# refresh-bio/KMC

Measured on AMD Instinct MI355X. Metric: stage-2 Gk-mers/s, k=27, higher is better.
Workload: dtype u64

## Files before the change

### kmc_amd/csrc/bucket_sort.hip.h

```cpp
#ifndef KMC_AMD_BUCKET_SORT_HIP_H
#define KMC_AMD_BUCKET_SORT_HIP_H

#include "kernels.hip.h"

#ifndef BR_NARROW_LOOP
#define BR_NARROW_LOOP 2
#endif
#ifndef BR_WIDE_LOOP
#define BR_WIDE_LOOP 1
#endif
#ifndef BR_WIDE_STEP
#define BR_WIDE_STEP 8
#endif
#ifndef BR_SLACK_DIV
#define BR_SLACK_DIV 12
#endif
#ifndef BR_INDIRECT_MIN_SIZE
#define BR_INDIRECT_MIN_SIZE 2
#endif
#ifndef BR_MIN_WAVES
#define BR_MIN_WAVES 6
#endif
template <int SIZE> __device__ __forceinline__ u64 bs_p64(const u64 (&x)[SIZE], u32 key_bits)
{
// ... 759 lines not shown
						s_aux[j] = (u32)kmc_remove_suffix<1>(kx, pshift) & lut_mask;
				}
				__syncthreads();
				for (u32 w = tid; w < ndw; w += THREADS) {
					const u32 i0 = w << 2;
					u32 ri = rec_bytes > 1 ? __umulhi(i0, inv) : i0, q = i0 - ri * rec_bytes;
					u64 cur = s_key[ri];
					u32 word = 0;
#pragma unroll
					for (int t = 0; t < 4; ++t) {
						word |= ((u32)(cur >> (8 * q)) & 0xFFu) << (8 * t);
						if (++q == rec_bytes) {
							q = 0;
							++ri;
							cur = s_key[ri < (u32)CAP ? ri : (u32)CAP - 1];
						}
					}
					dst32[w] = word;
				}
				if (use_lut) {
					u64 *lut = gr.lut_base[bin] + (size_t)(slot % lut_shards) * lut_stride;
					for (u32 j = tid; j < tile_counted; j += THREADS) {
						const u32 pf = s_aux[j];
						if (j + 1 == tile_counted || s_aux[j + 1] != pf)
							atomicAdd(&lut[pf], (u64)(j + 1));
						if (j > 0 && s_aux[j - 1] != pf)
							atomicAdd(&lut[pf], (u64)0 - (u64)j);
					}
				}
			} else {
#pragma unroll
				for (int r = 0; r < ITEMS; ++r) {
					const u32 rk16 = (rank2[r >> 1] >> ((r & 1) * 16)) & 0xFFFFu;
					if (rk16 != 0xFFFFu) {
						const u32 rank = wave_off + rk16;
						u64 kx[SIZE];
#pragma unroll
						for (int w = 0; w < SIZE; ++w)
							kx[w] = key[r][w];
						kmc_mask_low<SIZE>(kx, 2 * P.k);
						store_rec<SIZE>(s_key + (size_t)rank * SIZE, kx);
						s_aux[rank] = cnt[r];
					}
				}
				__syncthreads();
				auto out_byte = [&](u32 i) -> u32 {
					const u32 ri = rec_bytes > 1 ? __umulhi(i, inv) : i, q = i - ri * rec_bytes;
					if (q < P.sbytes) {
						const u32 pbyte = P.sbytes - 1 - q;
						return (u32)(s_key[(size_t)ri * SIZE + (pbyte >> 3)] >> ((pbyte & 7) * 8)) & 0xFFu;
					}
					const u32 cq = q - P.sbytes;
					return (s_aux[ri] >> (8 * (P.kff ? (P.cbytes - 1 - cq) : cq))) & 0xFFu;
				};
#pragma clang loop unroll(disable) vectorize(disable)
				for (u32 wd = tid; wd < ndw; wd += THREADS) {
					const u32 i0 = wd * 4;
					u32 word = out_byte(i0);
					word |= (i0 + 1 < tile_bytes ? out_byte(i0 + 1) : 0u) << 8;
					word |= (i0 + 2 < tile_bytes ? out_byte(i0 + 2) : 0u) << 16;
					word |= (i0 + 3 < tile_bytes ? out_byte(i0 + 3) : 0u) << 24;
					dst32[wd] = word;
				}
				if (use_lut) {
					u64 *lut = gr.lut_base[bin] + (size_t)(slot % lut_shards) * lut_stride;
					auto prefix_of = [&](u32 j) -> u32 {
						u64 x[SIZE];
						load_rec<SIZE>(s_key + (size_t)j * SIZE, x);
						return (u32)kmc_remove_suffix<SIZE>(x, pshift) & lut_mask;
					};
					for (u32 j = tid; j < tile_counted; j += THREADS) {
						const u32 pf = prefix_of(j);
						if (j + 1 == tile_counted || prefix_of(j + 1) != pf)
							atomicAdd(&lut[pf], (u64)(j + 1));
						if (j > 0 && prefix_of(j - 1) != pf)
							atomicAdd(&lut[pf], (u64)0 - (u64)j);
					}
				}
			}
		}
	}
}

template <int SIZE, bool FUSED>
__global__ void __launch_bounds__(BrCfg<SIZE>::THREADS, BR_MIN_WAVES) k_bucket_rank(const GrpRank gr, DevParams P, u32 key_bits, u32 hbits, u32 lut_shards, u64 lut_stride,
                                                                                  u32 lut_mask, u32 *flag)
{
	KMC_DYN_LDS(unsigned char, s_raw);
	br_tile<SIZE, FUSED>(gr, P, key_bits, hbits, lut_shards, lut_stride, lut_mask, flag, blockIdx.x, blockIdx.y, s_raw);
}

template <int SIZE>
__global__ void __launch_bounds__(GT_THREADS) k_giant_tiles(const GrpRank gr, DevParams P, u32 stride, u32 key_bits, u32 hbits, u32 lut_shards, u64 lut_stride, u32 lut_mask,
                                                              u32 *err )
{
	constexpr int THREADS = GT_THREADS, ITEMS = SIZE == 1 ? 8 : (SIZE == 2 ? 4 : 2), NW = THREADS / 64, CHUNK = THREADS * ITEMS;
	constexpr u32 NONE = 0xFFFFFFFFu;
	static_assert(THREADS >= 256, "one digit per thread");
	__shared__ u32 s_whist[NW * 256];
	__shared__ u32 s_base[256];
	__shared__ u32 s_scan[NW + 1];
	__shared__ u32 s_pick;
	__shared__ u32 s_wlast[NW], s_wcnt[NW];
	const u32 tid = threadIdx.x, lane = tid & 63;
	const u32 wave = (u32)__builtin_amdgcn_readfirstlane((int)(tid >> 6));
	const u32 rec_bytes = P.sbytes + P.cbytes;
	const bool use_lut = P.lut_prefix_len != 0 && !P.kff && !P.without_output;
	const u32 pshift = 2 * (P.k - P.lut_prefix_len);
	const u32 bsh = 64 - hbits, rbits = key_bits - hbits;
	const u64 lane_lt = (1ull << lane) - 1;
	while (true) {
		__syncthreads();
		if (tid == 0)
			s_pick = atomicAdd(&gr.giant[1], 1u);
		__syncthreads();
		const u32 pick = s_pick;
		if (pick >= ld_agent(&gr.giant[0]))
			break;
		const u32 entry = gr.giant[2 + pick];
		const u32 gtile = entry & ((1u << GT_CUT_SHIFT) - 1u), cut = entry >> GT_CUT_SHIFT;
		const u32 bin = (u32)__builtin_amdgcn_readfirstlane((int)grp_find(gr.win_prefix, gr.g, gtile));
		const u32 tile = gtile - gr.win_prefix[bin];
		const u64 b0 = gr.bounds[bin][tile] + cut, b1 = gr.bounds[bin][tile + 1];
		const u32 L = (u32)(b1 - b0);
		u64 *T = gr.S[bin] + b0 * SIZE;
		if (gr.rec_base) {
			T = gr.giant_T[bin] + b0 * SIZE;
			const u64 *pairs = gr.S[bin] + b0;
			for (u32 i = tid; i < L; i += THREADS) {
				u64 x[SIZE];
				load_rec<SIZE>(gr.rec_base + (size_t)(u32)pairs[i] * SIZE, x);
				store_rec<SIZE>(T + (size_t)i * SIZE, x);
			}
			__syncthreads();
		}
		u64 *U = reinterpret_cast<u64 *>(gr.scratch[bin] + b0 * (u64)(SIZE * 8));
		(void)stride;
		u32 passes;
		{
			u64 x0[SIZE], xl[SIZE];
			load_rec<SIZE>(T, x0);
			load_rec<SIZE>(T + (size_t)(L - 1) * SIZE, xl);
			const u64 k0 = hbits ? bs_p64<SIZE>(x0, key_bits) >> bsh : 0ull, kl = hbits ? bs_p64<SIZE>(xl, key_bits) >> bsh : 0ull;
			const u64 diff = k0 ^ kl;
			const u32 dbits = diff ? 64u - (u32)__clzll((long long)diff) : 0u;
			const u32 nbits = rbits + dbits < key_bits ? rbits + dbits : key_bits;
			passes = (nbits + 7) / 8;
		}
		u64 *src = T, *dst = U;
		for (u32 p = 0; p < passes; ++p) {
			if (tid < 256)
				s_base[tid] = 0;
			__syncthreads();
			for (u32 i = tid; i < L; i += THREADS) {
				u64 x[SIZE];
				load_rec<SIZE>(src + (size_t)i * SIZE, x);
				(void)__hip_atomic_fetch_add(&s_base[kmc_get_byte<SIZE>(x, p)], 1u, __ATOMIC_RELAXED, __HIP_MEMORY_SCOPE_WORKGROUP);
			}
			__syncthreads();
			{
				const u32 v = tid < 256 ? s_base[tid] : 0u;
				u32 total;
				const u32 ex = block_excl_sum<NW, u32>(v, s_scan, total);
				if (tid < 256)
					s_base[tid] = ex;
			}
			__syncthreads();
			for (u32 c0 = 0; c0 < L; c0 += CHUNK) {
				for (u32 i = tid; i < (u32)NW * 256; i += THREADS)
					s_whist[i] = 0;
				__syncthreads();
				u64 key[ITEMS][SIZE];
// ... 188 lines not shown
```

### kmc_amd/csrc/host_plan_and_groups.hip.h

```cpp
u32 lut_shards_for(u64 lut_entries) { return lut_entries <= 256 ? 32u : (lut_entries <= 1024 ? 8u : 1u); }

struct BinPlan {
	const uint8_t *d_in = nullptr;
	u64 size = 0, n_rec = 0, n_packs = 0;
	const u64 *d_pack_start = nullptr;
	uint8_t *d_out = nullptr;
	u64 out_capacity = 0;
	u64 *d_out_bytes = nullptr, *d_lut = nullptr, *d_stats = nullptr;
	size_t off_bitmap = 0, off_exp_status = 0, off_cp_status = 0, off_lutsh = 0, off_tally = 0;
	u64 rec_off = 0;
};

struct SortPlan {
	u32 key_bytes = 0, top = 0;
	u32 key_bits = 0;
	bool rank = false;
	u32 pass_lo() const { return key_bytes - top; }
	bool local() const { return top < key_bytes; }
	u32 hbits() const { return top ? 8 * top - (8 * key_bytes - key_bits) : 0; }
};
std::atomic<u64> g_path[4] = {};
std::atomic<u64> g_indirect_groups{0};
std::atomic<u64> g_hybrid_groups{0}, g_redo_groups{0};
std::atomic<u32> g_extra_top{0};
// ... 57 lines not shown
	if (n <= (u64)BrCfg<SIZE>::THREADS * (8 / SIZE > 2 ? 8 / SIZE : 2))
		return sp;
	const u64 redo = g_redo_groups.load(std::memory_order_relaxed);
	if (g_extra_top.load(std::memory_order_relaxed) >= 2 && redo > 128 && redo * 8 > g_hybrid_groups.load(std::memory_order_relaxed))
		return sp;
	for (u32 h = 1; h + 2 <= key_bytes && h <= 6u; ++h) {
		const u32 eff = 8 * h > spare ? 8 * h - spare : 0;
		if (eff >= 28 && (eff >= 63 || (n >> eff) <= 2) && key_bits - eff <= rem_limit) {
			sp.top = h;
			break;
		}
	}
	if (sp.top + 2 > key_bytes)
		sp.top = key_bytes;
	static const int forced = [] {
		const char *e = getenv("KMC_HIP_RANK_TOP");
		return e ? atoi(e) : 0;
	}();
	if (forced >= 1 && (u32)forced + 1 <= key_bytes && 8 * (u32)forced > spare)
		sp.top = (u32)forced;
	if (sp.local() && sp.top >= 1 && key_bits - sp.hbits() <= rem_limit && sp.hbits() <= 48)
		sp.rank = true;
	else
		sp.top = key_bytes;
	return sp;
}

template <int SIZE>
ZeroPlan plan_group(const Slot &s, std::vector<BinPlan> &bins, u64 n_total, u32 n_pass , bool front, bool sort, bool compact, u64 lut_shard_entries,
                    u64 cp_tile = CpCfg<SIZE>::TILE ,
                    u32 cp_words = 1 , u64 giant_entries = 0, bool arena = false)
{
	ZeroPlan z;
	size_t off = up256(SM_BYTES);
	if (giant_entries) {
		z.giant = off;
		off += up256((size_t)(giant_entries + 2) * 4);
	}
	if (arena) {
		z.arena = off;
		off += up256((size_t)AR_DYN_WORDS * 4) + up256((size_t)AR_MAX_PASS * 256 * 8);
	}
	for (BinPlan &b : bins) {
		if (front) {
			b.off_bitmap = off;
			off += up256(((b.size + 31) / 32 + 2) * 4);
			b.off_exp_status = off;
			off += up256(((b.size + EXP_CHUNK - 1) / EXP_CHUNK) * 8 + 8);
		}
		if (compact) {
			b.off_cp_status = off;
			off += up256(((b.n_rec + cp_tile - 1) / cp_tile) * 8 * cp_words + 8);
			b.off_lutsh = off;
			off += up256(lut_shard_entries * 8);
			b.off_tally = off;
			off += up256(CP_SHARDS * 4 * 8);
		}
	}
	if (front || sort) {
		z.ghist = off;
		off += up256((size_t)n_pass * 256 * 8);
	}
	if (sort && n_total >= 2) {
		const u64 max_tiles = (std::min(n_total, s.portion) + RsCfg<SIZE>::TILE - 1) / RsCfg<SIZE>::TILE;
		const u64 n_launch = (u64)n_pass * ((n_total + s.portion - 1) / s.portion);
		z.sc_status = off;
		z.sc_stride = up256((size_t)max_tiles * 256 * 4);
		off += z.sc_stride * n_launch;
	}
	z.total = off;
	return z;
}

int apply_plan(Slot &s, const ZeroPlan &z)
{
	s.zero_grew = z.total > s.zero.cap;
	++s.groups_run;
	if (int rc = ensure(s.zero, z.total))
		return rc;
	HIPCHK(hipMemsetAsync(s.zero.p, 0, z.total, s.stream));
	return 0;
}

template <int SIZE>
int sort_device_t(Slot &s, const ZeroPlan &z, u64 *d_recs, u64 *d_tmp, u64 n, const SortPlan &sp, u64 **d_result, u32 &counter_idx, bool hist_done, u32 *d_flag,
                  bool local_by_caller = false )
{
	u64 *src = d_recs, *dst = d_tmp;
	if (n < 2 || sp.key_bytes == 0) {
		*d_result = src;
		if (s.timed)
			HIPCHK(hipEventRecord(s.ev[3], s.stream));
		return 0;
	}
	const u32 n_pass = sp.top, pass_lo = sp.pass_lo();
	u32 *err = err_ptr(s);
	if (n_pass) {
		if (int rc = ensure(s.dbase, (size_t)n_pass * 256 * 8))
			return rc;
		u64 *ghist = zero_ptr<u64>(s, z.ghist), *dbase = (u64 *)s.dbase.p;
		u32 *counters = small_ptr<u32>(s, SM_COUNTERS);
		u64 *work = small_ptr<u64>(s, SM_DBASE_WORK);

		if (!hist_done) {
			u64 blocks = (n + 255) / 256;
			if (blocks > 256 * 8)
				blocks = 256 * 8;
			k_hist<SIZE><<<dim3((u32)blocks), dim3(256), (size_t)n_pass * 1024, s.stream>>>(src, n, n_pass, ghist, pass_lo);
			k_hist_scan<<<dim3(n_pass), dim3(256), 0, s.stream>>>(ghist, dbase);
		}
		if (s.timed)
			HIPCHK(hipEventRecord(s.ev[3], s.stream));
		u32 launch = 0;
		for (u32 pass = 0; pass < n_pass; ++pass) {
			const u64 *base_in = dbase + (size_t)pass * 256;
			int flip = 0;
			for (u64 start = 0; start < n; start += s.portion) {
				const u32 cnt = (u32)std::min(s.portion, n - start);
				const u32 tiles = (cnt + RsCfg<SIZE>::TILE - 1) / RsCfg<SIZE>::TILE;
				if (counter_idx >= N_COUNTERS)
					return fail(KMC_HIP_EINVAL, "too many scatter launches for one bin");
				u32 *status = zero_ptr<u32>(s, z.sc_status + (size_t)launch * z.sc_stride);
				u64 *base_out = work + (size_t)flip * 256;
				hipEvent_t e0 = nullptr, e1 = nullptr;
				if (s.timed) {
					if (int rc = sc_event_pair(s, e0, e1, cnt))
						return rc;
					HIPCHK(hipEventRecord(e0, s.stream));
				}
				static const size_t scatter_pad = [] {
					const char *e = getenv("KMC_HIP_SCATTER_LDS_PAD");
					const size_t v = e ? (size_t)strtoull(e, nullptr, 10) : (size_t)0;
					return v > 32 * 1024 ? (size_t)32 * 1024 : v;
				}();
				k_onesweep<SIZE><<<dim3((tiles + RS_TPB - 1) / RS_TPB), dim3(RS_BLOCK), rs_lds_bytes<SIZE>() + scatter_pad, s.stream>>>(
				    src + start * SIZE, dst, cnt, pass_lo + pass, base_in, base_out, status, counters + counter_idx, tiles, err);
				if (s.timed)
					HIPCHK(hipEventRecord(e1, s.stream));
				++counter_idx;
				++launch;
				base_in = base_out;
				flip ^= 1;
			}
			std::swap(src, dst);
		}
	} else if (s.timed)
		HIPCHK(hipEventRecord(s.ev[3], s.stream));
	if (sp.local() && !local_by_caller) {
		if constexpr (SIZE == 1) {
			if (!sp.rank)
				return fail(KMC_HIP_EINTERNAL, "a local sort plan without the rank finisher");
			const u64 S = (u64)BrCfg<1>::STRIDE;
			const u64 n_win = (n + S - 1) / S;
			if (n_win > 0x7FFFFFF0ull)
				return fail(KMC_HIP_EINVAL, "bin too large");
			if (int rc = ensure(s.bounds, (size_t)(n_win + 2) * 8))
				return rc;
			u64 *bounds = (u64 *)s.bounds.p;
			hipEvent_t e0 = nullptr, e1 = nullptr;
			if (s.timed) {
				if (int rc = ls_event_pair(s, e0, e1, n))
					return rc;
				HIPCHK(hipEventRecord(e0, s.stream));
			}
			GrpBounds gbn = {};
			gbn.g = 1;
			gbn.item_prefix[1] = (u32)(n_win + 1);
			gbn.S[0] = src;
			gbn.n[0] = n;
			gbn.bounds[0] = bounds;
			k_bucket_bounds<1><<<dim3((u32)((n_win + 1 + 3) / 4)), dim3(256), 0, s.stream>>>(gbn, (u32)S, sp.key_bits, sp.hbits());
			GrpRank gr = {};
			gr.g = 1;
			gr.win_prefix[1] = (u32)n_win;
			gr.S[0] = src;
			gr.bounds[0] = bounds;
			k_bucket_rank<1, false><<<dim3((u32)n_win, 2), dim3(BrCfg<1>::THREADS), br_lds_bytes<1>(), s.stream>>>(gr, DevParams{}, sp.key_bits, sp.hbits(), 1u, 0ull, 0u, d_flag);
			if (s.timed)
				HIPCHK(hipEventRecord(e1, s.stream));
		} else
			return fail(KMC_HIP_EINTERNAL, "records of two words and more have no in-place local sort");
	}
	HIPCHK(hipGetLastError());
	*d_result = src;
	return 0;
}

template <int SIZE> int sort_only_t(Slot &s, u64 *d_recs, u64 *d_tmp, u64 n, u32 key_bytes, u64 **d_result, bool stable_lsd)
{
	std::vector<BinPlan> none;
	const SortPlan sp = plan_sort<SIZE>(n, key_bytes, 8 * key_bytes, stable_lsd);
	const ZeroPlan z = plan_group<SIZE>(s, none, n, sp.top, false, true, false, 0);
	if (int rc = apply_plan(s, z))
		return rc;
	u32 counter_idx = 0;
	return sort_device_t<SIZE>(s, z, d_recs, d_tmp, n, sp, d_result, counter_idx, false, small_ptr<u32>(s, SM_REDO));
}

int sort_device(Slot &s, u64 *d_recs, u64 *d_tmp, u64 n, u32 words, u32 n_pass, u64 **d_result, bool stable_lsd)
{
	return by_words<8>(words, [&](auto W) { return sort_only_t<decltype(W)::value>(s, d_recs, d_tmp, n, n_pass, d_result, stable_lsd); });
}

int check_params(const kmc_hip_bin_params *p, DevParams &P)
{
	if (!p)
		return fail(KMC_HIP_EINVAL, "params == NULL");
	if (p->kmer_len < 1 || p->kmer_len > 256)
		return fail(KMC_HIP_EINVAL, "kmer_len must be 1..256");
	if (p->output_type > 1)
		return fail(KMC_HIP_EINVAL, "output_type must be 0 (KMC) or 1 (KFF)");
	if (p->lut_prefix_len >= p->kmer_len && p->lut_prefix_len)
		return fail(KMC_HIP_EINVAL, "lut_prefix_len must be < kmer_len");
	if (p->lut_prefix_len > 15)
		return fail(KMC_HIP_EINVAL, "lut_prefix_len must be <= 15");
	if (p->lut_prefix_len && (p->kmer_len - p->lut_prefix_len) % 4)
		return fail(KMC_HIP_EINVAL, "(kmer_len - lut_prefix_len) must be a multiple of 4 (kmc.h:1454-1456)");
	P.k = p->kmer_len;
	P.both_strands = p->both_strands ? 1 : 0;
	P.cutoff_min = p->cutoff_min;
	P.cutoff_max = (u32)p->cutoff_max;
	P.counter_max = (u32)p->counter_max;
	P.lut_prefix_len = p->lut_prefix_len;
	P.sbytes = kmc_suffix_bytes(p->kmer_len, p->lut_prefix_len);
	P.cbytes = counter_bytes(p->cutoff_max, p->counter_max);
	P.kff = p->output_type == 1;
	P.without_output = p->without_output ? 1 : 0;
	return 0;
}

template <int SIZE>
int front_end_group(Slot &s, const std::vector<BinPlan> &bins, size_t off_ghist, const DevParams &P, u32 n_pass , u32 pass_lo, u32 &counter_idx,
                    bool &hist_done, u64 *d_recs, bool fuse, u64 *d_pairs = nullptr )
{
	if (bins.empty())
		return 0;
	if (bins.size() > (size_t)GRP_MAX)
		return fail(KMC_HIP_EINVAL, "group too large");
	u32 *err = err_ptr(s);
	u32 *counters = small_ptr<u32>(s, SM_COUNTERS);
	if (counter_idx + 2 > N_COUNTERS)
		return fail(KMC_HIP_EINVAL, "too many launches for one bin");
	GrpParse gp = {};
	GrpExpand ge = {};
	gp.g = ge.g = (u32)bins.size();
	u64 packs = 0, chunks = 0;
	const u32 tag_shift = (2 * P.k) & 63;
	for (size_t i = 0; i < bins.size(); ++i) {
		const BinPlan &b = bins[i];
		gp.pack_prefix[i] = (u32)packs;
		ge.chunk_prefix[i] = (u32)chunks;
		packs += b.n_packs;
		chunks += (b.size + EXP_CHUNK - 1) / EXP_CHUNK;
		if (packs > 0x7FFFFFF0ull || chunks > 0x7FFFFFF0ull)
			return fail(KMC_HIP_EINVAL, "bin too large");
		gp.data[i] = ge.data[i] = b.d_in;
		gp.pack_start[i] = b.d_pack_start;
		gp.bitmap[i] = zero_ptr<u32>(s, b.off_bitmap);
		ge.bitmap[i] = gp.bitmap[i];
		ge.size[i] = b.size;
// ... 9 lines not shown
	u64 *ghist = zero_ptr<u64>(s, off_ghist);
	k_parse_packs<<<dim3((u32)packs), dim3(PARSE_BLOCK), 0, s.stream>>>(gp, P.k, err);
	if (s.timed)
		HIPCHK(hipEventRecord(s.ev[1], s.stream));
	const u32 blocks = (u32)std::min<u64>(chunks, 256 * 4 * (512 / EXP_BLOCK));
	if (fuse) {
		if (int rc = ensure(s.dbase, (size_t)n_pass * 256 * 8))
			return rc;
		k_expand<SIZE, true><<<dim3(blocks), dim3(EXP_BLOCK), exp_lds_bytes<true>(n_pass, P.k), s.stream>>>(
		    ge, P.k, P.both_strands, n_pass, ghist, counters + counter_idx, err, (u64 *)s.dbase.p, counters + counter_idx + 1, pass_lo);
	} else
		k_expand<SIZE, false><<<dim3(blocks), dim3(EXP_BLOCK), exp_lds_bytes<false>(n_pass, P.k), s.stream>>>(
		    ge, P.k, P.both_strands, n_pass, ghist, counters + counter_idx, err, nullptr, counters + counter_idx + 1, pass_lo);
	counter_idx += 2;
	hist_done = fuse;
	if (s.timed)
		HIPCHK(hipEventRecord(s.ev[2], s.stream));
	HIPCHK(hipGetLastError());
	return 0;
}

template <int SIZE>
int compact_group(Slot &s, const std::vector<BinPlan> &bins, const u64 *sorted, u64 *scratch, const DevParams &P, u64 lut_entries, u32 &counter_idx)
{
	if (bins.empty())
		return 0;
	u32 *err = err_ptr(s);
	u32 *counters = small_ptr<u32>(s, SM_COUNTERS);
	if (counter_idx >= N_COUNTERS)
		return fail(KMC_HIP_EINVAL, "too many launches for one bin");
	const bool use_lut = lut_entries && !P.without_output && !P.kff;
	const u32 n_sh = !use_lut ? 1u : lut_shards_for(lut_entries);
	const u32 rec_bytes = P.sbytes + P.cbytes;
	const u64 tile_pitch = (u64)CpCfg<SIZE>::TILE * SIZE * 8;
	static const bool allow_two_phase = [] {
		const char *e = getenv("KMC_HIP_TWO_PHASE");
		return !e || atoi(e) != 0;
	}();
	const bool two_phase = allow_two_phase && scratch && !P.without_output &&
	                       ((u64)CpCfg<SIZE>::TILE / std::max<u32>(P.cutoff_min, 1) + 1) * rec_bytes <= tile_pitch;
	GrpCompact gc = {};
	GrpFold gf = {};
	GrpGather gg = {};
	gc.g = gg.g = (u32)bins.size();
	u64 tiles = 0;
	for (size_t i = 0; i < bins.size(); ++i) {
		const BinPlan &b = bins[i];
		gc.tile_prefix[i] = gg.tile_prefix[i] = (u32)tiles;
		const u64 bin_tiles = (b.n_rec + CpCfg<SIZE>::TILE - 1) / CpCfg<SIZE>::TILE;
		tiles += bin_tiles;
		if (tiles > 0x7FFFFFFFull)
			return fail(KMC_HIP_EINVAL, "bin too large");
		u64 *lut_base = b.d_lut;
		if (use_lut && n_sh > 1)
			lut_base = zero_ptr<u64>(s, b.off_lutsh);
		else if (lut_entries && !P.kff && b.d_lut)
			HIPCHK(hipMemsetAsync(b.d_lut, 0, lut_entries * 8, s.stream));
		gc.S[i] = sorted + b.rec_off * SIZE;
		gc.n[i] = gf.n[i] = b.n_rec;
		gc.out[i] = b.d_out;
		gc.out_capacity[i] = b.out_capacity;
		gc.lut_base[i] = lut_base;
		gc.tally[i] = zero_ptr<u64>(s, b.off_tally);
		gc.out_bytes[i] = b.d_out_bytes;
		gc.status[i] = zero_ptr<u64>(s, b.off_cp_status);
		gf.tally[i] = gc.tally[i];
		gf.stats[i] = b.d_stats;
		gf.lut_base[i] = lut_base;
		gf.lut_out[i] = b.d_lut;
		gc.scratch[i] = two_phase ? (uint8_t *)(scratch + b.rec_off * SIZE) : nullptr;
		gf.status[i] = gc.status[i];
		gf.n_tiles[i] = (u32)bin_tiles;
		gf.out_bytes[i] = b.d_out_bytes;
		gf.out_capacity[i] = b.out_capacity;
		gg.scratch[i] = gc.scratch[i];
		gg.prefix[i] = gc.status[i];
		gg.out[i] = b.d_out;
		gg.out_capacity[i] = b.out_capacity;
	}
	gc.tile_prefix[bins.size()] = gg.tile_prefix[bins.size()] = (u32)tiles;
	k_compact<SIZE><<<dim3((u32)tiles), dim3(CP_BLOCK), 0, s.stream>>>(gc, P, n_sh, lut_entries, counters + counter_idx, err,
	                                                                   P.lut_prefix_len ? (u32)((1ull << (2 * P.lut_prefix_len)) - 1) : 0u, two_phase ? 1u : 0u);
	counter_idx += 1;
	k_compact_fold<<<dim3((u32)bins.size()), dim3(256), 0, s.stream>>>(gf, use_lut ? n_sh : 1u, lut_entries, two_phase ? 1u : 0u, rec_bytes, err);
	if (two_phase)
		k_compact_gather<<<dim3((u32)((tiles + 3) / 4)), dim3(256), 0, s.stream>>>(gg, rec_bytes, tile_pitch);
	HIPCHK(hipGetLastError());
	return 0;
}

template <int SIZE> bool count_applicable(const DevParams &P)
{
	static const bool allow_two_phase = [] {
		const char *e = getenv("KMC_HIP_TWO_PHASE");
		return !e || atoi(e) != 0;
	}();
	const u32 rec_bytes = P.sbytes + P.cbytes;
	return allow_two_phase && (P.without_output || rec_bytes <= (u32)(SIZE * 8));
}
template <int SIZE>
int rank_group(Slot &s, const std::vector<BinPlan> &bins, u64 *sorted, u64 *scratch, const DevParams &P, u64 lut_entries, const SortPlan &sp, u64 n_total, u32 *d_flag,
               u32 *d_giant, const u64 *d_recs_indirect = nullptr ,
               u32 *d_arena = nullptr )
{
	if (bins.empty())
		return 0;
	u32 *err = err_ptr(s);
	const bool use_lut = lut_entries && !P.without_output && !P.kff;
	const u32 n_sh = !use_lut ? 1u : lut_shards_for(lut_entries);
	const u32 rec_bytes = P.sbytes + P.cbytes;
	constexpr u64 S = BrCfg<SIZE>::STRIDE;
	GrpBounds gbn = {};
	GrpRank gr = {};
	GrpFold gf = {};
	GrpGather gg = {};
	gbn.g = gr.g = gg.g = (u32)bins.size();
	u64 wins = 0, items = 0;
	for (const BinPlan &b : bins) {
		items += (b.n_rec + S - 1) / S + 1;
		wins += (b.n_rec + S - 1) / S;
	}
	if (items > 0x3FFFFFF0ull)
		return fail(KMC_HIP_EINVAL, "bin too large");
	if (int rc = ensure(s.bounds, (size_t)(items + 2 + 2 * wins) * 8))
		return rc;
	u64 *bounds = (u64 *)s.bounds.p, *chunk_src = bounds + items + 2;
	items = wins = 0;
	for (size_t i = 0; i < bins.size(); ++i) {
		const BinPlan &b = bins[i];
		const u64 bin_wins = (b.n_rec + S - 1) / S;
		gbn.item_prefix[i] = (u32)items;
		gr.win_prefix[i] = (u32)wins;
		gg.tile_prefix[i] = (u32)(2 * wins);
		u64 *lut_base = b.d_lut;
		if (use_lut && n_sh > 1)
			lut_base = zero_ptr<u64>(s, b.off_lutsh);
		else if (lut_entries && !P.kff && b.d_lut)
			HIPCHK(hipMemsetAsync(b.d_lut, 0, lut_entries * 8, s.stream));
		gbn.S[i] = sorted + b.rec_off * (d_recs_indirect ? 1 : SIZE);
		gr.S[i] = sorted + b.rec_off * (d_recs_indirect ? 1 : SIZE);
		gbn.n[i] = gf.n[i] = b.n_rec;
		gbn.bounds[i] = bounds + items;
		gr.bounds[i] = bounds + items;
		gr.scratch[i] = (uint8_t *)(scratch + b.rec_off * SIZE);
		gr.giant_T[i] = d_recs_indirect ? (u64 *)s.recC.p + b.rec_off * SIZE : nullptr;
		gr.status[i] = zero_ptr<u64>(s, b.off_cp_status);
		gr.chunk_src[i] = chunk_src + 2 * wins;
		gr.lut_base[i] = lut_base;
		gr.tally[i] = zero_ptr<u64>(s, b.off_tally);
		gf.tally[i] = gr.tally[i];
		gf.stats[i] = b.d_stats;
		gf.lut_base[i] = lut_base;
		gf.lut_out[i] = b.d_lut;
		gf.status[i] = gr.status[i];
		gf.n_tiles[i] = (u32)(2 * bin_wins);
		gf.out_bytes[i] = b.d_out_bytes;
		gf.out_capacity[i] = b.out_capacity;
		gg.scratch[i] = gr.scratch[i];
		gg.prefix[i] = gr.status[i];
		gg.out[i] = b.d_out;
		gg.out_capacity[i] = b.out_capacity;
		gg.src_rec[i] = gr.chunk_src[i];
		items += bin_wins + 1;
		wins += bin_wins;
	}
	gbn.item_prefix[bins.size()] = (u32)items;
	gr.win_prefix[bins.size()] = (u32)wins;
// ... 163 lines not shown
						}
				}
				dbg_prev.swap(cur);
				return 0;
			};
			if (debug_steps)
				if (int rc = debug_step(-1))
					return rc;
			for (u32 pass = 0; pass < ar_pass_max; ++pass) {
				if (debug_steps && pass)
					if (int rc = debug_step((int)pass - 1))
						return rc;
				static const bool debug_static = getenv("KMC_HIP_ARENA_DEBUG") && atoi(getenv("KMC_HIP_ARENA_DEBUG")) >= 3;
				if (debug_static) {
					HIPCHK(hipStreamSynchronize(s.stream));
					u32 h_dyn[AR_DYN_WORDS];
					HIPCHK(hipMemcpy(h_dyn, dyn, sizeof h_dyn, hipMemcpyDeviceToHost));
					if (h_dyn[AR_M] && pass < h_dyn[AR_N_PASS]) {
						const u32 tiles = (h_dyn[AR_M] + RsCfg<1>::TILE - 1) / RsCfg<1>::TILE;
						k_onesweep<1><<<dim3(tiles), dim3(RS_BLOCK), rs_lds_bytes<1>(), s.stream>>>((pass & 1u) ? aw.B : aw.A, (pass & 1u) ? aw.A : aw.B, h_dyn[AR_M], pass,
						                                                                         aw.dbase + (size_t)pass * 256, aw.dbase + (size_t)AR_MAX_PASS * 256,
						                                                                         aw.status + (size_t)pass * aw.status_stride, dyn + AR_PASS_TICKET + pass, tiles, err);
					}
					continue;
				}
				k_onesweep_dyn<1><<<dim3(g_sweep), dim3(RS_BLOCK), rs_lds_bytes<1>(), s.stream>>>((pass & 1u) ? aw.B : aw.A, (pass & 1u) ? aw.A : aw.B, dyn + AR_M, pass,
				                                                                                  aw.dbase + (size_t)pass * 256, aw.dbase + (size_t)AR_MAX_PASS * 256,
				                                                                                  aw.status + (size_t)pass * aw.status_stride, dyn + AR_PASS_TICKET + pass, err);
			}
			if (debug_steps)
				if (int rc = debug_step((int)ar_pass_max - 1))
					return rc;
			static const bool debug = getenv("KMC_HIP_ARENA_DEBUG") != nullptr;
			if (debug) {
				HIPCHK(hipStreamSynchronize(s.stream));
				u32 h_dyn[AR_DYN_WORDS];
				HIPCHK(hipMemcpy(h_dyn, dyn, sizeof h_dyn, hipMemcpyDeviceToHost));
				const u32 M = h_dyn[AR_M], ne = h_dyn[AR_N_ENT], np = h_dyn[AR_N_PASS];
				fprintf(stderr, "[arena debug] entries %u records %u passes %u (max %u) items %u heavy %u overflow %u rbits %u\n", ne, M, np, ar_pass_max, h_dyn[AR_N_ITEMS], 0u,
				        h_dyn[AR_OVERFLOW], rbits);
				if (M) {
					std::vector<u64> ar(M);
					std::vector<u32> off(ne + 1);
					std::vector<ArenaEntry> ent(ne);
					HIPCHK(hipMemcpy(ar.data(), (np & 1u) ? aw.B : aw.A, (size_t)M * 8, hipMemcpyDeviceToHost));
					HIPCHK(hipMemcpy(off.data(), aw.arena_off, (size_t)(ne + 1) * 4, hipMemcpyDeviceToHost));
					HIPCHK(hipMemcpy(ent.data(), gr.arena_ent, (size_t)ne * sizeof(ArenaEntry), hipMemcpyDeviceToHost));
					u64 inversions = 0, first_inv = ~0ull;
					for (u32 i = 1; i < M; ++i)
						if (ar[i - 1] > ar[i]) {
							if (!inversions)
								first_inv = i;
							++inversions;
						}
					u64 bad_entries = 0, first_bad = ~0ull, bad_ord = 0;
					const u64 rmask = rbits >= 64 ? ~0ull : ((1ull << rbits) - 1);
					std::vector<u64> slice;
					for (u32 e = 0; e < ne; ++e) {
						const u64 gpos = ent[e].w0 & ((1ull << 40) - 1);
						slice.resize(ent[e].len);
						HIPCHK(hipMemcpy(slice.data(), aw.S0 + gpos, (size_t)ent[e].len * 8, hipMemcpyDeviceToHost));
						for (auto &x : slice)
							x = ((u64)e << rbits) | (x & rmask);
						std::sort(slice.begin(), slice.end());
						bool ok = off[e + 1] - off[e] == ent[e].len;
						for (u32 i = 0; ok && i < ent[e].len; ++i)
							ok = ar[off[e] + i] == slice[i];
						for (u32 i = off[e]; i < off[e + 1] && i < M; ++i)
							if ((ar[i] >> rbits) != e)
								++bad_ord;
						if (!ok) {
							if (!bad_entries)
								first_bad = e;
							++bad_entries;
						}
					}
					fprintf(stderr, "[arena debug] inversions %llu (first at %llu), entries whose slice is not their bucket in order: %llu (first %llu), records under a foreign ordinal %llu\n",
					        (unsigned long long)inversions, (unsigned long long)first_inv, (unsigned long long)bad_entries, (unsigned long long)first_bad, (unsigned long long)bad_ord);
				}
			}
			k_arena_finish<<<dim3(g_finish * (AR_THREADS / AF_THREADS)), dim3(AF_THREADS), 0, s.stream>>>(gr, aw, P, rbits, n_sh, lut_entries, lut_mask, err);
		}
	}
	k_bucket_rank<SIZE, true><<<dim3((u32)wins, 2), dim3(BrCfg<SIZE>::THREADS), br_lds_bytes<SIZE>() + lds_pad, s.stream>>>(gr, P, sp.key_bits, sp.hbits(), n_sh, lut_entries, lut_mask, d_flag);
	if (!arena_ran && giant_list)
		k_giant_tiles<SIZE><<<dim3((u32)std::min<u64>(wins, 256 * (1024 / GT_THREADS))), dim3(GT_THREADS), 0, s.stream>>>(gr, P, (u32)S, sp.key_bits, sp.hbits(), n_sh, lut_entries, lut_mask, err);
	if (s.timed)
		HIPCHK(hipEventRecord(e1, s.stream));
	k_compact_fold<<<dim3((u32)bins.size()), dim3(256), 0, s.stream>>>(gf, use_lut ? n_sh : 1u, lut_entries, 1u, rec_bytes, err);
	if (!P.without_output)
		k_compact_gather<<<dim3((u32)((2 * wins + 3) / 4)), dim3(256), 0, s.stream>>>(gg, rec_bytes, (u64)SIZE * 8);
	HIPCHK(hipGetLastError());
	return 0;
}

u32 group_capacity(u32 k, bool small_bins)
{
	static const int limit = [] {
		const char *e = getenv("KMC_HIP_GROUP");
		const int v = e ? atoi(e) : GRP_MAX;
		return v < 1 ? 1 : (v > GRP_MAX ? GRP_MAX : v);
	}();
	const u32 words = (k + 31) / 32;
	const u32 spare = 8 * ((2 * k + 7) / 8) - 2 * k;
	const u32 room = 64 * words - 2 * k;
	const u32 bits = small_bins ? (room > 4 ? 4 : room) : (spare > 4 ? 4 : spare);
	const u32 cap = 1u << bits;
	return cap < (u32)limit ? cap : (u32)limit;
}
constexpr u64 GROUP_SMALL_BIN_RECORDS = 2ull << 20;
constexpr u64 GROUP_MAX_RECORD_BYTES = 6ull << 30;
#ifndef INDIRECT_MIN_WORDS
#define INDIRECT_MIN_WORDS 2
#endif

template <int SIZE>
int run_group_device_t(Slot &s, const DevParams &P, const kmc_hip_bin_desc *const *descs, u32 g, u64 lut_entries, bool classic, u32 *d_flag, bool *used_hybrid)
{
	const u32 k = P.k;
	const bool use_lut = lut_entries && !P.without_output && !P.kff;
	const u32 n_sh = use_lut ? lut_shards_for(lut_entries) : 1u;
	std::vector<BinPlan> bins;
	u64 N = 0;
	for (u32 i = 0; i < g; ++i) {
		const kmc_hip_bin_desc &d = *descs[i];
		if ((d.n_rec == 0) != (d.size == 0))
			return fail(KMC_HIP_ECORRUPT, "exactly one of size / n_rec is zero");
		if (d.n_rec == 0)
			continue;
		if (d.n_packs == 0 || d.n_packs > 0xFFFFFFF0ull)
			return fail(KMC_HIP_EINVAL, "n_packs out of range");
		BinPlan b;
		b.d_in = d.d_superkmers;
		b.size = d.size;
		b.n_rec = d.n_rec;
		b.n_packs = d.n_packs;
		b.d_pack_start = (const u64 *)d.d_pack_start;
		b.d_out = d.d_out;
		b.out_capacity = d.out_capacity;
		b.d_out_bytes = (u64 *)d.d_out_bytes;
		b.d_lut = (u64 *)d.d_lut;
		b.d_stats = (u64 *)d.d_stats;
		b.rec_off = N;
		N += d.n_rec;
		bins.push_back(b);
	}
	u32 tag_bits = 0;
	while ((1u << tag_bits) < bins.size())
		++tag_bits;
	if (2 * k + tag_bits > 64u * SIZE)
		return fail(KMC_HIP_EINVAL, "group too large for the record width");
	const u32 key_bytes = (2 * k + tag_bits + 7) / 8;
	static const bool fuse_enabled = [] {
		const char *e = getenv("KMC_HIP_RANK_FUSE");
		return !e || atoi(e) != 0;
	}();
	const bool can_fuse = count_applicable<SIZE>(P);
	const bool by_rank = !classic && hybrid_mode() == 1 && rank_enabled() && (SIZE == 1 || (can_fuse && fuse_enabled));
	const SortPlan sp = plan_sort<SIZE>(N, key_bytes, 2 * k + tag_bits, !by_rank, by_rank);
	const bool rank_fused = sp.rank && can_fuse && fuse_enabled;
	const u32 n_pass = sp.top;
	if (used_hybrid)
		*used_hybrid = sp.local() && N >= 2;
	const bool fuse = n_pass >= 1 && n_pass <= EXP_FUSE_MAX_PASS && N >= 2;
	static const bool indirect_enabled = [] {
		const char *e = getenv("KMC_HIP_INDIRECT");
		return !e || atoi(e) != 0;
	}();
	bool indirect = SIZE >= INDIRECT_MIN_WORDS && indirect_enabled && rank_fused && sp.local() && n_pass == 4 && fuse && N < (1ull << 32);
	int rc = 0;
	if (N && ((rc = ensure(s.recA, N * SIZE * 8 + 256)) || (rc = ensure(s.recB, N * SIZE * 8 + 256))))
		return rc;
// ... 233 lines not shown
```

### kmc_amd/csrc/kernels.hip.h

```cpp
#ifndef KMC_AMD_KERNELS_HIP_H
#define KMC_AMD_KERNELS_HIP_H

#include <hip/hip_runtime.h>
#include <stdint.h>

#include <type_traits>
#include "kmer_ops.h"

typedef kmc_u64 u64;
typedef kmc_u32 u32;

#ifndef KMC_DYN_LDS
#define KMC_DYN_LDS(type, name) extern __shared__ __attribute__((aligned(16))) type name[]
#define KMC_LAUNDER(x) asm volatile("" : "+v"(x))
#define KMC_WAIT_VMEM() asm volatile("s_waitcnt vmcnt(0)" ::: "memory")
#define KMC_WAVE_LOCKSTEP() ((void)0)
#endif

enum : u32 { KERR_CORRUPT = 1u, KERR_NREC = 2u, KERR_CAPACITY = 4u,
             KERR_WATCHDOG = 8u,
             KERR_PEER = 0x10u,
             KERR_AT_SCATTER = 0x100u, KERR_AT_EXPAND = 0x200u, KERR_AT_COMPACT = 0x400u, KERR_AT_STAGE1 = 0x800u };
constexpr int KERR_DIAG_WORDS = 11;

// ... 1445 lines not shown
					__syncthreads();
				}
			} else {
				for (u32 c0 = 0; c0 < tile_bytes; c0 += CP_STAGE) {
					const u32 c1 = (tile_bytes - c0) < (u32)CP_STAGE ? tile_bytes : c0 + CP_STAGE;
#pragma unroll
					for (int r = 0; r < ROWS; ++r) {
						const u32 rk16 = (rank2[r >> 1] >> ((r & 1) * 16)) & 0xFFFFu;
						if (rk16 != 0xFFFFu) {
							const u32 rank = wave_off + rk16;
							if (use_lut && c0 == 0)
								s_pref[rank] = (u32)kmc_remove_suffix<SIZE>(key[r], pshift) & lut_mask;
							const u32 bb = rank * rec_bytes;
							if (bb < c1 && bb + rec_bytes > c0) {
								for (u32 q = 0; q < rec_bytes; ++q) {
									const u32 bpos = bb + q;
									if (bpos >= c0 && bpos < c1) {
										u32 val;
										if (q < P.sbytes)
											{
												const u32 pb = P.sbytes - 1 - q, top = 2 * P.k;
												val = kmc_get_byte<SIZE>(key[r], pb);
												if (8 * pb + 8 > top)
													val = top > 8 * pb ? (val & ((1u << (top - 8 * pb)) - 1)) : 0u;
											}
										else {
											const u32 cq = q - P.sbytes;
											val = cnt[r] >> (8 * (P.kff ? (P.cbytes - 1 - cq) : cq));
										}
										s_stage[bpos - c0] = (uint8_t)val;
									}
								}
							}
						}
					}
					__syncthreads();
					const u64 gbyte0 = two_phase ? 0 : s_tile_off * rec_bytes;
					const bool fits = two_phase || gbyte0 + tile_bytes <= out_capacity;
					if (!fits && tid == 0)
						atomicOr(err, KERR_CAPACITY);
					if (fits) {
						const u64 g0 = gbyte0 + c0;
						const u32 len = c1 - c0;
						u32 head = (u32)((4 - ((uintptr_t)(dst + g0) & 3)) & 3);
						if (head > len)
							head = len;
						const u32 ndw = (len - head) >> 2;
						const u32 tail0 = head + (ndw << 2);
						if (tid < head)
							dst[g0 + tid] = s_stage[tid];
						if (tid >= 32 && tid - 32 < len - tail0)
							dst[g0 + tail0 + (tid - 32)] = s_stage[tail0 + (tid - 32)];
						u32 *gd = reinterpret_cast<u32 *>(dst + g0 + head);
						for (u32 w = tid; w < ndw; w += CP_BLOCK) {
							const uint8_t *sp = s_stage + head + (w << 2);
							gd[w] = (u32)sp[0] | ((u32)sp[1] << 8) | ((u32)sp[2] << 16) | ((u32)sp[3] << 24);
						}
					}
					__syncthreads();
				}
			}
			if (use_lut) {
				u64 *lut = lut_base + (size_t)(tile % lut_shards) * lut_stride;
				for (u32 j = tid; j < tile_counted; j += CP_BLOCK) {
					const u32 pf = s_pref[j];
					if (j + 1 == tile_counted || s_pref[j + 1] != pf)
						atomicAdd(&lut[pf], (u64)(j + 1));
					if (j > 0 && s_pref[j - 1] != pf)
						atomicAdd(&lut[pf], (u64)0 - (u64)j);
				}
			}
		}
		TRACE_STAMP(1, tile, 7);
	}
}

__global__ void __launch_bounds__(256) k_compact_fold(const GrpFold gf, u32 lut_shards, u64 lut_stride, u32 two_phase, u32 rec_bytes, u32 *err)
{
	const u32 bin = blockIdx.x;
	const u64 *__restrict__ stat_shards = gf.tally[bin];
	u64 *__restrict__ stats = gf.stats[bin];
	const u64 *__restrict__ lut_base = gf.lut_base[bin];
	u64 *__restrict__ lut_out = gf.lut_out[bin];
	if (threadIdx.x < 64) {
		const u32 lane = threadIdx.x;
		for (int j = 0; j < 3; ++j) {
			u64 v = lane < CP_SHARDS ? stat_shards[lane * 4 + j] : 0;
			v = wave_sum<u64>(v);
			if (lane == 0)
				stats[j] = v;
		}
		if (lane == 0)
			stats[3] = gf.n[bin];
	}
	if (two_phase) {
		__shared__ u64 s_scan[5];
		u64 *st = gf.status[bin];
		const u32 nt = gf.n_tiles[bin];
		constexpr u32 CH = CP_FOLD_CHUNK, PER = CH / 256;
		static_assert(CH % 256 == 0 && CH >= 256, "CP_FOLD_CHUNK");
		__shared__ u64 s_buf[CH];
		u64 carry = 0;
		for (u32 c0 = 0; c0 < nt; c0 += CH) {
			const u32 cn = (nt - c0) < CH ? (nt - c0) : CH;
			for (u32 i = threadIdx.x; i < CH; i += 256)
				s_buf[i] = i < cn ? st[c0 + i] : 0;
			__syncthreads();
			u64 sum = 0;
#pragma unroll
			for (u32 j = 0; j < PER; ++j)
				sum += s_buf[threadIdx.x * PER + j];
			u64 total;
			u64 run = carry + block_excl_sum<4, u64>(sum, s_scan, total);
#pragma unroll
			for (u32 j = 0; j < PER; ++j) {
				const u64 v = s_buf[threadIdx.x * PER + j];
				s_buf[threadIdx.x * PER + j] = run;
				run += v;
			}
			__syncthreads();
			for (u32 i = threadIdx.x; i < cn; i += 256)
				st[c0 + i] = s_buf[i];
			carry += total;
			__syncthreads();
		}
		if (threadIdx.x == 0) {
			st[nt] = carry;
			*gf.out_bytes[bin] = carry * rec_bytes;
			if (carry * rec_bytes > gf.out_capacity[bin])
				atomicOr(err, KERR_CAPACITY);
		}
	}
	if (lut_shards > 1) {
		for (u64 i = threadIdx.x; i < lut_stride; i += 256) {
			u64 v = 0;
			for (u32 s0 = 0; s0 < lut_shards; s0 += 8) {
				u64 part[8];
#pragma unroll
				for (int q = 0; q < 8; ++q)
					part[q] = (s0 + q < lut_shards) ? lut_base[(size_t)(s0 + q) * lut_stride + i] : 0ull;
#pragma unroll
				for (int q = 0; q < 8; ++q)
					v += part[q];
			}
			lut_out[i] = v;
		}
	}
}

__global__ void __launch_bounds__(256) k_compact_gather(const GrpGather gg, u32 rec_bytes, u64 tile_pitch)
{
	const u32 lane = threadIdx.x & 63;
	const u32 gtile = blockIdx.x * 4 + (threadIdx.x >> 6);
	if (gtile >= gg.tile_prefix[gg.g])
		return;
	const u32 bin = grp_find(gg.tile_prefix, gg.g, gtile);
	const u32 tile = gtile - gg.tile_prefix[bin];
	const u32 nt = gg.tile_prefix[bin + 1] - gg.tile_prefix[bin];
	const u64 *__restrict__ prefix = gg.prefix[bin];
	if (prefix[nt] * rec_bytes > gg.out_capacity[bin])
		return;
	const u64 first = prefix[tile];
	const u32 len = (u32)(prefix[tile + 1] - first) * rec_bytes;
	if (!len)
		return;
	const uint8_t *__restrict__ src = gg.scratch[bin] + (gg.src_rec[bin] ? gg.src_rec[bin][tile] : (u64)tile) * tile_pitch;
	uint8_t *__restrict__ dst = gg.out[bin] + first * rec_bytes;
	u32 head = (u32)((4 - ((uintptr_t)dst & 3)) & 3);
	if (head > len)
		head = len;
	const u32 ndw = (len - head) >> 2, tail0 = head + (ndw << 2);
	if (lane < head)
		dst[lane] = src[lane];
	if (lane >= 32 && lane - 32 < len - tail0)
		dst[tail0 + lane - 32] = src[tail0 + lane - 32];
	const u32 *__restrict__ s32 = reinterpret_cast<const u32 *>(src);
	u32 *__restrict__ d32 = reinterpret_cast<u32 *>(dst + head);
	const u32 sh = 8 * head;
	for (u32 w = lane; w < ndw; w += 64) {
		const u32 lo = s32[w];
		const u32 hi = head ? s32[w + 1] : 0;
		d32[w] = head ? ((lo >> sh) | (hi << (32 - sh))) : lo;
	}
}

#endif
```

### kmc_amd/csrc/kmc_hip.hip

```cpp
#include <hip/hip_runtime.h>
#include <rccl/rccl.h>

#include <algorithm>
#include <atomic>
#include <chrono>
#include <cstdint>
#include <cstdio>
#include <cstdlib>
#include <cstring>
#include <memory>
#include <condition_variable>
#include <mutex>
#include <string>
#include <thread>
#include <type_traits>
#include <vector>

#include "../../include/kmc_hip.h"
#include "kernels.hip.h"
#include "bucket_sort.hip.h"
#include "arena_sort.hip.h"
#include "order_db.hip.h"
#include "stage1_kernels.hip.h"
#include "count_gather.hip.h"
// ... 185 lines not shown
	std::condition_variable idle;
};
struct AccumHold {
	Accum *a = nullptr;
	void take(Accum &acc)
	{
		++acc.users;
		a = &acc;
	}
	~AccumHold()
	{
		if (!a)
			return;
		std::lock_guard<std::mutex> lck(a->mtx);
		if (--a->users == 0)
			a->idle.notify_all();
	}
};

struct Dev {
	int ordinal = 0;
	u32 rr = 0;
	std::mutex rr_mtx;
	Slot slot[N_SLOTS];
	DBuf rccl_buf;
	DBuf xchg;
	int *d_sig_map = nullptr;
	u32 sig_map_entries = 0;
	std::mutex map_mtx;
	DBuf s1_arena[N_SLOTS];
	Accum est;
	Accum smallk;
};

u32 counter_bytes(u64 cutoff_max, u64 counter_max) { return kmc_counter_bytes(cutoff_max, counter_max); }

}

struct kmc_hip_ctx {
	std::vector<std::unique_ptr<Dev>> devs;
	std::vector<ncclComm_t> comms;
	bool comms_ready = false;
	u64 portion = PORTION_MAX;
	std::mutex mtx;
	std::vector<struct kmc_hip_count *> counts;
};

namespace {

template <int MAX, int W = 1, class F> int by_words(u32 words, F &&f)
{
	if (words == (u32)W)
		return f(std::integral_constant<int, W>{});
	if constexpr (W < MAX)
		return by_words<MAX, W + 1>(words, f);
	else
		return fail(KMC_HIP_EINVAL, "records of " + std::to_string(words) + " words: this entry takes 1.." + std::to_string(MAX));
}

u32 env_positive(const char *name, u32 dflt)
{
	const char *e = getenv(name);
	return e && atoi(e) > 0 ? (u32)atoi(e) : dflt;
}

int set_dev(kmc_hip_ctx *ctx, int dev)
{
	if (!ctx || dev < 0 || dev >= (int)ctx->devs.size())
		return fail(KMC_HIP_EINVAL, "bad ctx/dev");
	HIPCHK(hipSetDevice(ctx->devs[dev]->ordinal));
	return 0;
}

template <int SIZE> int set_func_attrs()
{
	if (rs_lds_bytes<SIZE>() + 32 * 1024 > 65536 && rs_lds_bytes<SIZE>() + 32 * 1024 <= 160 * 1024)
		HIPCHK(hipFuncSetAttribute(reinterpret_cast<const void *>(&k_onesweep<SIZE>), hipFuncAttributeMaxDynamicSharedMemorySize,
		                           (int)rs_lds_bytes<SIZE>() + 32 * 1024));
	else if (rs_lds_bytes<SIZE>() > 65536)
		HIPCHK(hipFuncSetAttribute(reinterpret_cast<const void *>(&k_onesweep<SIZE>), hipFuncAttributeMaxDynamicSharedMemorySize,
		                           (int)rs_lds_bytes<SIZE>()));
	if (br_lds_bytes<SIZE>() > 65536) {
		HIPCHK(hipFuncSetAttribute(reinterpret_cast<const void *>(&k_bucket_rank<SIZE, true>), hipFuncAttributeMaxDynamicSharedMemorySize, (int)br_lds_bytes<SIZE>() + 32 * 1024));
		if (SIZE == 1) {
			HIPCHK(hipFuncSetAttribute(reinterpret_cast<const void *>(&k_bucket_rank<1, false>), hipFuncAttributeMaxDynamicSharedMemorySize, (int)br_lds_bytes<1>()));
		}
	}
	if (exp_lds_bytes<true>(EXP_FUSE_MAX_PASS, 1) > 65536)
		HIPCHK(hipFuncSetAttribute(reinterpret_cast<const void *>(&k_expand<SIZE, true>), hipFuncAttributeMaxDynamicSharedMemorySize,
		                           (int)exp_lds_bytes<true>(EXP_FUSE_MAX_PASS, 1)));
	return 0;
}
int set_all_func_attrs()
{
	for (u32 words = 1; words <= 8; ++words)
		if (int rc = by_words<8>(words, [](auto W) { return set_func_attrs<decltype(W)::value>(); }))
			return rc;
	return 0;
}

int slot_init(Slot &s, u64 portion)
{
	s.portion = portion;
	HIPCHK(hipStreamCreateWithFlags(&s.stream, hipStreamNonBlocking));
	HIPCHK(hipHostMalloc((void **)&s.h_hb_res, sizeof(HbRes), hipHostMallocDefault));
	memset(s.h_hb_res, 0, sizeof(HbRes));
	if (int rc = ensure(s.hb_res, sizeof(HbRes)))
		return rc;
	for (auto &e : s.ev)
		HIPCHK(hipEventCreate(&e));
	HIPCHK(hipEventCreateWithFlags(&s.done_ev, hipEventBlockingSync | hipEventDisableTiming));
	if (int rc = ensure(s.zero, SM_BYTES))
		return rc;
	HIPCHK(hipMemset(s.zero.p, 0, SM_BYTES));
	if (int rc = ensure(s.sticky, 256))
		return rc;
	HIPCHK(hipMemset(s.sticky.p, 0, 256));
	return 0;
}

void slot_destroy(Slot &s)
{
	for (DBuf *b : {&s.in, &s.pack_start, &s.recA, &s.recB, &s.recC, &s.pairA, &s.pairB, &s.zero, &s.dbase, &s.out, &s.lut, &s.sticky, &s.bounds, &s.arena_work, &s.redo_log, &s.hb_res})
		if (b->p && !b->carved)
			(void)hipFree(b->p);
	if (s.slab.p)
		(void)hipFree(s.slab.p);
	if (s.h_hb_res)
		(void)hipHostFree(s.h_hb_res);
	if (s.h_stage_in)
		(void)hipHostFree(s.h_stage_in);
	if (s.h_stage_out)
		(void)hipHostFree(s.h_stage_out);
	for (auto &e : s.ev)
		if (e)
			(void)hipEventDestroy(e);
	for (auto &e : s.sc_ev)
		(void)hipEventDestroy(e);
	if (s.done_ev)
		(void)hipEventDestroy(s.done_ev);
	if (s.stream)
		(void)hipStreamDestroy(s.stream);
}

template <typename T> T *small_ptr(Slot &s, size_t off) { return reinterpret_cast<T *>(static_cast<char *>(s.zero.p) + off); }
template <typename T> T *zero_ptr(Slot &s, size_t off) { return reinterpret_cast<T *>(static_cast<char *>(s.zero.p) + off); }
u32 *err_ptr(Slot &s) { return static_cast<u32 *>(s.sticky.p); }

int sc_event_pair(Slot &s, hipEvent_t &e0, hipEvent_t &e1, u64 cnt)
{
	while (s.sc_ev.size() < (size_t)s.sc_used + 2) {
		hipEvent_t ne;
		HIPCHK(hipEventCreate(&ne));
		s.sc_ev.push_back(ne);
	}
	e0 = s.sc_ev[s.sc_used];
	e1 = s.sc_ev[s.sc_used + 1];
	s.sc_used += 2;
	s.sc_cnt.push_back(cnt);
	return 0;
}

int ls_event_pair(Slot &s, hipEvent_t &e0, hipEvent_t &e1, u64 cnt) { return sc_event_pair(s, e0, e1, cnt | (1ull << 63)); }

int harvest(Slot &s)
{
	for (u32 i = 0; i + 1 < s.sc_used; i += 2) {
		float t = 0;
// ... 169 lines not shown
```

Before: 35.24.

## Replace 2-D bucket-rank grid with sparse follow-up kernel and parallelize LUT fold

The bucket-rank launch no longer uses a second grid-y slice per window. A new k_bucket_rank_rest kernel scans the window bounds, ballots for windows longer than the tile capacity, and runs the second tile only for those. This avoids launching many idle y=1 workgroups, at the cost of an extra kernel launch and serialized processing of long windows inside each block. Separately, k_compact_fold moves its LUT shard reduction into extra grid-y workgroups (up to 16) so it runs in parallel with the per-bin prefix work instead of after it in a single block.

Result: no change. 34.93 (-0.9%).

```diff
diff --git a/kmc_amd/csrc/bucket_sort.hip.h b/kmc_amd/csrc/bucket_sort.hip.h
--- a/kmc_amd/csrc/bucket_sort.hip.h
+++ b/kmc_amd/csrc/bucket_sort.hip.h
@@ -865,12 +865,50 @@
 	}
 }
 
+#ifndef BR_GRID_Y2
+#define BR_GRID_Y2 0
+#endif
 template <int SIZE, bool FUSED>
 __global__ void __launch_bounds__(BrCfg<SIZE>::THREADS, BR_MIN_WAVES) k_bucket_rank(const GrpRank gr, DevParams P, u32 key_bits, u32 hbits, u32 lut_shards, u64 lut_stride,
                                                                                   u32 lut_mask, u32 *flag)
 {
 	KMC_DYN_LDS(unsigned char, s_raw);
 	br_tile<SIZE, FUSED>(gr, P, key_bits, hbits, lut_shards, lut_stride, lut_mask, flag, blockIdx.x, blockIdx.y, s_raw);
+}
+
+template <int SIZE, bool FUSED>
+__global__ void __launch_bounds__(BrCfg<SIZE>::THREADS, BR_MIN_WAVES) k_bucket_rank_rest(const GrpRank gr, DevParams P, u32 key_bits, u32 hbits, u32 lut_shards, u64 lut_stride,
+                                                                                       u32 lut_mask, u32 *flag, u32 n_tiles)
+{
+	KMC_DYN_LDS(unsigned char, s_raw);
+	constexpr int THREADS = BrCfg<SIZE>::THREADS, NW = BrCfg<SIZE>::NW;
+	__shared__ u64 s_long[NW];
+	const u32 lane = threadIdx.x & 63, wave = threadIdx.x >> 6;
+	for (u64 base = (u64)blockIdx.x * THREADS; base < n_tiles; base += (u64)gridDim.x * THREADS) {
+		const u64 t = base + threadIdx.x;
+		bool is_long = false;
+		if (t < n_tiles) {
+			const u32 bin = grp_find(gr.win_prefix, gr.g, (u32)t);
+			const u64 *bounds = gr.bounds[bin];
+			const u32 tile = (u32)t - gr.win_prefix[bin];
+			is_long = bounds[tile + 1] - bounds[tile] > (u64)BrCfg<SIZE>::CAP;
+		}
+		const u64 m = __ballot(is_long);
+		if (lane == 0)
+			s_long[wave] = m;
+		__syncthreads();
+#pragma clang loop unroll(disable)
+		for (int w = 0; w < NW; ++w) {
+			u64 left = wave_first(s_long[w]);
+			while (left) {
+				const u32 i = (u32)__ffsll((long long)left) - 1u;
+				left &= left - 1;
+				br_tile<SIZE, FUSED>(gr, P, key_bits, hbits, lut_shards, lut_stride, lut_mask, flag, (u32)base + (u32)w * 64u + i, 1u, s_raw);
+				__syncthreads();
+			}
+		}
+		__syncthreads();
+	}
 }
 
 template <int SIZE>
diff --git a/kmc_amd/csrc/host_plan_and_groups.hip.h b/kmc_amd/csrc/host_plan_and_groups.hip.h
--- a/kmc_amd/csrc/host_plan_and_groups.hip.h
+++ b/kmc_amd/csrc/host_plan_and_groups.hip.h
@@ -163,6 +163,10 @@
 	return 0;
 }
 
+template <int SIZE> dim3 br_rest_grid(u64 tiles)
+{
+	return dim3((u32)std::min<u64>((tiles + BrCfg<SIZE>::THREADS - 1) / BrCfg<SIZE>::THREADS, 256 * 2));
+}
 template <int SIZE>
 int sort_device_t(Slot &s, const ZeroPlan &z, u64 *d_recs, u64 *d_tmp, u64 n, const SortPlan &sp, u64 **d_result, u32 &counter_idx, bool hist_done, u32 *d_flag,
                   bool local_by_caller = false )
@@ -256,7 +260,10 @@
 			gr.win_prefix[1] = (u32)n_win;
 			gr.S[0] = src;
 			gr.bounds[0] = bounds;
-			k_bucket_rank<1, false><<<dim3((u32)n_win, 2), dim3(BrCfg<1>::THREADS), br_lds_bytes<1>(), s.stream>>>(gr, DevParams{}, sp.key_bits, sp.hbits(), 1u, 0ull, 0u, d_flag);
+			k_bucket_rank<1, false><<<dim3((u32)n_win, BR_GRID_Y2 ? 2 : 1), dim3(BrCfg<1>::THREADS), br_lds_bytes<1>(), s.stream>>>(gr, DevParams{}, sp.key_bits, sp.hbits(), 1u, 0ull, 0u, d_flag);
+			if (!BR_GRID_Y2)
+				k_bucket_rank_rest<1, false><<<br_rest_grid<1>(n_win), dim3(BrCfg<1>::THREADS), br_lds_bytes<1>(), s.stream>>>(gr, DevParams{}, sp.key_bits, sp.hbits(), 1u, 0ull, 0u, d_flag,
+				                                                                                                          (u32)n_win);
 			if (s.timed)
 				HIPCHK(hipEventRecord(e1, s.stream));
 		} else
@@ -432,7 +439,7 @@
 	k_compact<SIZE><<<dim3((u32)tiles), dim3(CP_BLOCK), 0, s.stream>>>(gc, P, n_sh, lut_entries, counters + counter_idx, err,
 	                                                                   P.lut_prefix_len ? (u32)((1ull << (2 * P.lut_prefix_len)) - 1) : 0u, two_phase ? 1u : 0u);
 	counter_idx += 1;
-	k_compact_fold<<<dim3((u32)bins.size()), dim3(256), 0, s.stream>>>(gf, use_lut ? n_sh : 1u, lut_entries, two_phase ? 1u : 0u, rec_bytes, err);
+	k_compact_fold<<<cp_fold_grid((u32)bins.size(), use_lut ? n_sh : 1u, lut_entries), dim3(256), 0, s.stream>>>(gf, use_lut ? n_sh : 1u, lut_entries, two_phase ? 1u : 0u, rec_bytes, err);
 	if (two_phase)
 		k_compact_gather<<<dim3((u32)((tiles + 3) / 4)), dim3(256), 0, s.stream>>>(gg, rec_bytes, tile_pitch);
 	HIPCHK(hipGetLastError());
@@ -762,12 +769,15 @@
 			k_arena_finish<<<dim3(g_finish * (AR_THREADS / AF_THREADS)), dim3(AF_THREADS), 0, s.stream>>>(gr, aw, P, rbits, n_sh, lut_entries, lut_mask, err);
 		}
 	}
-	k_bucket_rank<SIZE, true><<<dim3((u32)wins, 2), dim3(BrCfg<SIZE>::THREADS), br_lds_bytes<SIZE>() + lds_pad, s.stream>>>(gr, P, sp.key_bits, sp.hbits(), n_sh, lut_entries, lut_mask, d_flag);
+	k_bucket_rank<SIZE, true><<<dim3((u32)wins, BR_GRID_Y2 ? 2 : 1), dim3(BrCfg<SIZE>::THREADS), br_lds_bytes<SIZE>() + lds_pad, s.stream>>>(gr, P, sp.key_bits, sp.hbits(), n_sh, lut_entries, lut_mask, d_flag);
+	if (!BR_GRID_Y2)
+		k_bucket_rank_rest<SIZE, true><<<br_rest_grid<SIZE>(wins), dim3(BrCfg<SIZE>::THREADS), br_lds_bytes<SIZE>(), s.stream>>>(gr, P, sp.key_bits, sp.hbits(), n_sh, lut_entries, lut_mask, d_flag,
+		                                                                                                                    (u32)wins);
 	if (!arena_ran && giant_list)
 		k_giant_tiles<SIZE><<<dim3((u32)std::min<u64>(wins, 256 * (1024 / GT_THREADS))), dim3(GT_THREADS), 0, s.stream>>>(gr, P, (u32)S, sp.key_bits, sp.hbits(), n_sh, lut_entries, lut_mask, err);
 	if (s.timed)
 		HIPCHK(hipEventRecord(e1, s.stream));
-	k_compact_fold<<<dim3((u32)bins.size()), dim3(256), 0, s.stream>>>(gf, use_lut ? n_sh : 1u, lut_entries, 1u, rec_bytes, err);
+	k_compact_fold<<<cp_fold_grid((u32)bins.size(), use_lut ? n_sh : 1u, lut_entries), dim3(256), 0, s.stream>>>(gf, use_lut ? n_sh : 1u, lut_entries, 1u, rec_bytes, err);
 	if (!P.without_output)
 		k_compact_gather<<<dim3((u32)((2 * wins + 3) / 4)), dim3(256), 0, s.stream>>>(gg, rec_bytes, (u64)SIZE * 8);
 	HIPCHK(hipGetLastError());
diff --git a/kmc_amd/csrc/kernels.hip.h b/kmc_amd/csrc/kernels.hip.h
--- a/kmc_amd/csrc/kernels.hip.h
+++ b/kmc_amd/csrc/kernels.hip.h
@@ -1551,6 +1551,26 @@
 	u64 *__restrict__ stats = gf.stats[bin];
 	const u64 *__restrict__ lut_base = gf.lut_base[bin];
 	u64 *__restrict__ lut_out = gf.lut_out[bin];
+	if (blockIdx.y != 0 || gridDim.y == 1) {
+		if (lut_shards > 1) {
+			const u32 lut_wgs = gridDim.y > 1 ? gridDim.y - 1 : 1u, lut_wg = gridDim.y > 1 ? blockIdx.y - 1 : 0u;
+			for (u64 i = (u64)lut_wg * 256 + threadIdx.x; i < lut_stride; i += (u64)lut_wgs * 256) {
+				u64 v = 0;
+				for (u32 s0 = 0; s0 < lut_shards; s0 += 8) {
+					u64 part[8];
+#pragma unroll
+					for (int q = 0; q < 8; ++q)
+						part[q] = (s0 + q < lut_shards) ? lut_base[(size_t)(s0 + q) * lut_stride + i] : 0ull;
+#pragma unroll
+					for (int q = 0; q < 8; ++q)
+						v += part[q];
+				}
+				lut_out[i] = v;
+			}
+		}
+		if (blockIdx.y != 0)
+			return;
+	}
 	if (threadIdx.x < 64) {
 		const u32 lane = threadIdx.x;
 		for (int j = 0; j < 3; ++j) {
@@ -1600,21 +1620,16 @@
 				atomicOr(err, KERR_CAPACITY);
 		}
 	}
-	if (lut_shards > 1) {
-		for (u64 i = threadIdx.x; i < lut_stride; i += 256) {
-			u64 v = 0;
-			for (u32 s0 = 0; s0 < lut_shards; s0 += 8) {
-				u64 part[8];
-#pragma unroll
-				for (int q = 0; q < 8; ++q)
-					part[q] = (s0 + q < lut_shards) ? lut_base[(size_t)(s0 + q) * lut_stride + i] : 0ull;
-#pragma unroll
-				for (int q = 0; q < 8; ++q)
-					v += part[q];
-			}
-			lut_out[i] = v;
-		}
-	}
+}
+#ifndef CP_FOLD_LUT_WGS
+#define CP_FOLD_LUT_WGS 16
+#endif
+inline dim3 cp_fold_grid(u32 bins, u32 lut_shards, u64 lut_stride)
+{
+	u64 f = lut_shards > 1 ? (lut_stride + 255) / 256 : 0;
+	if (f > CP_FOLD_LUT_WGS)
+		f = CP_FOLD_LUT_WGS;
+	return dim3(bins, 1 + (u32)f);
 }
 
 __global__ void __launch_bounds__(256) k_compact_gather(const GrpGather gg, u32 rec_bytes, u64 tile_pitch)
diff --git a/kmc_amd/csrc/kmc_hip.hip b/kmc_amd/csrc/kmc_hip.hip
--- a/kmc_amd/csrc/kmc_hip.hip
+++ b/kmc_amd/csrc/kmc_hip.hip
@@ -291,8 +291,10 @@
 		                           (int)rs_lds_bytes<SIZE>()));
 	if (br_lds_bytes<SIZE>() > 65536) {
 		HIPCHK(hipFuncSetAttribute(reinterpret_cast<const void *>(&k_bucket_rank<SIZE, true>), hipFuncAttributeMaxDynamicSharedMemorySize, (int)br_lds_bytes<SIZE>() + 32 * 1024));
+		HIPCHK(hipFuncSetAttribute(reinterpret_cast<const void *>(&k_bucket_rank_rest<SIZE, true>), hipFuncAttributeMaxDynamicSharedMemorySize, (int)br_lds_bytes<SIZE>()));
 		if (SIZE == 1) {
 			HIPCHK(hipFuncSetAttribute(reinterpret_cast<const void *>(&k_bucket_rank<1, false>), hipFuncAttributeMaxDynamicSharedMemorySize, (int)br_lds_bytes<1>()));
+			HIPCHK(hipFuncSetAttribute(reinterpret_cast<const void *>(&k_bucket_rank_rest<1, false>), hipFuncAttributeMaxDynamicSharedMemorySize, (int)br_lds_bytes<1>()));
 		}
 	}
 	if (exp_lds_bytes<true>(EXP_FUSE_MAX_PASS, 1) > 65536)
```
